# yuansliu/minicom

Measured on AMD Instinct MI355X. Metric: Mreads/s (sketch+index+overlap) on 150bp reads, 1/2/4/8 GPU; bit-exact decompress, higher is better.
Workload: dtype u64

## Files before the change

minicom_amd/csrc/api.hip:

```cpp
#include "mcom_dev.hpp"
#include "../../include/mcom_test.h"
#include <stdarg.h>
#include <stdlib.h>
#include <cxxabi.h>
#include <stdio.h>
#include <string.h>

int mcom_fail(mcom_ctx *ctx, int code, const char *fmt, ...)
{
	char buf[512];
	va_list ap;
	va_start(ap, fmt);
	vsnprintf(buf, sizeof buf, fmt, ap);
	va_end(ap);
	if (ctx) { ctx->err = buf; ctx->pin_wait.clear(); ctx->pin_off = 0; }
	return code;
}

#define MCOM_PIN_BYTES 4096
hipError_t mcom_d2h_async(mcom_ctx *ctx, void *dst, const void *src, size_t bytes)
{
	for (uint32_t q = 0; q < 8; ++q) {
		const mcom_ctx::ScanTotal &t = ctx->scan_last[(ctx->scan_last_at + 7u - q) % 8u];
		if (t.last && t.last == src && t.bytes == bytes && t.gen == ctx->launch_gen) { mcom_ctx::PinWait w{dst, 0, bytes}; w.from = ctx->scan_tot + t.slot; ctx->pin_wait.push_back(w); return hipSuccess; }
// ... 307 lines not shown
	if (!ctx) return MCOM_E_ARG;
	ctx->sketch_wave_only = wave_per_string == 1;
	ctx->sketch_ring64 = wave_per_string == 2;
	ctx->sketch_ring32_only = wave_per_string == 3;
	ctx->sketch_lane_always = wave_per_string >= 2;
	return MCOM_OK;
}
extern "C" int mcom_set_sketch_prefix_bits(mcom_ctx *ctx, int bits)
{
	if (!ctx || bits < 1 || bits > 30) return MCOM_E_ARG;
	ctx->sketch_prefix_bits = bits;
	return MCOM_OK;
}
extern "C" int mcom_set_claim_route(mcom_ctx *ctx, int route)
{
	if (!ctx || route < 0 || route > 3) return MCOM_E_ARG;
	ctx->claim_route = route;
	return MCOM_OK;
}
extern "C" int mcom_claim_fallbacks(const mcom_ctx *ctx) { return ctx ? (int)ctx->claim_fallbacks : 0; }
extern "C" int mcom_set_screen_route(mcom_ctx *ctx, int route)
{
	if (!ctx || route < 0 || route > 2) return MCOM_E_ARG;
	ctx->screen_route = route;
	return MCOM_OK;
}
extern "C" int mcom_screen_fallbacks(const mcom_ctx *ctx) { return ctx ? (int)ctx->screen_fallbacks : 0; }
extern "C" int mcom_set_lookup_route(mcom_ctx *ctx, int route)
{
	if (!ctx || route < 0 || route > 1) return MCOM_E_ARG;
	ctx->lookup_route = route;
	return MCOM_OK;
}
extern "C" int mcom_set_index_capacity(mcom_ctx *ctx, int entries)
{
	if (!ctx) return MCOM_E_ARG;
	ctx->cix_cap_set = entries >= 0; ctx->cix_cap = entries >= 0 ? (uint32_t)entries : 0u;
	return MCOM_OK;
}
```

minicom_amd/csrc/cindex.hip:

```cpp
#include "cindex.hpp"
#include <algorithm>

#define CX_THREADS 256
#define CX_ITEMS 24
#define CX_TILE (CX_THREADS * CX_ITEMS)

__global__ void k_cindex_blocks(int maxoff, const uint64_t *__restrict__ woff, uint32_t c0, uint32_t c1, uint64_t pos0, uint64_t n_blocks, uint32_t *__restrict__ first_contig)
{
	const uint32_t c = c0 + blockIdx.x * blockDim.x + threadIdx.x;
	if (c >= c1) return;
	const uint64_t a = woff[c] + (uint64_t)maxoff * c - pos0, b = woff[c + 1] + (uint64_t)maxoff * (c + 1) - pos0;
	for (uint64_t blk = (a + 255) >> 8; (blk << 8) < b && blk < n_blocks; ++blk) first_contig[blk] = c;
}

__device__ __forceinline__ uint32_t cx_tile(uint32_t b, uint32_t n_tiles) { const uint32_t per = (n_tiles + 7u) >> 3; return (b & 7u) * per + (b >> 3); }
static inline uint32_t cx_grid(uint32_t n_tiles) { return ((n_tiles + 7u) >> 3) << 3; }

struct CxSrc { const uint64_t *cbits, *coff, *woff; const uint32_t *first_contig; uint32_t c1; uint64_t pos0, n_pos; unsigned long long *head; };

struct CxWalk { uint32_t c; bool has; uint64_t p, np, lo, hi; };
__device__ __forceinline__ uint64_t cx_first(const CixGeom &g, const CxSrc &s, uint32_t c) { return s.woff[c] + (uint64_t)g.maxoff * c - s.pos0; }
__device__ __forceinline__ void cx_load(const CixGeom &g, const CxSrc &s, CxWalk &w)
{
	w.has = s.woff[w.c + 1] != s.woff[w.c];
	if (!w.has || w.p >= w.np) return;
	const uint64_t len = (s.woff[w.c + 1] - s.woff[w.c]) + (uint64_t)g.L - 1;
	const uint64_t q = (2 * len + 63) >> 6, i = (2 * w.p) >> 6;
	const uint64_t *src = s.cbits + s.coff[w.c] + i;
	const int sh = (int)((2 * w.p) & 63);
	const uint64_t w0 = src[0], w1 = src[1], w2 = i + 2 <= q ? src[2] : 0ull;
	w.lo = sh ? (w0 >> sh) | (w1 << (64 - sh)) : w0;
	w.hi = sh ? (w1 >> sh) | (w2 << (64 - sh)) : w1;
}
__device__ __forceinline__ void cx_seek(const CixGeom &g, const CxSrc &s, uint64_t gi, CxWalk &w)
{
	uint32_t c = s.first_contig[gi >> 8];
	while (c + 1 < s.c1 && cx_first(g, s, c + 1) <= gi) ++c;
	const uint64_t a = cx_first(g, s, c);
	w.c = c; w.p = gi - a; w.np = cx_first(g, s, c + 1) - a;
	cx_load(g, s, w);
}
__device__ __forceinline__ bool cx_step(const CixGeom &g, const CxSrc &s, CxWalk &w, uint32_t &key32, uint64_t &slot, uint32_t &digit)
{
	while (w.p >= w.np) {
		++w.c; w.p = 0; w.np = cx_first(g, s, w.c + 1) - cx_first(g, s, w.c);
		cx_load(g, s, w);
	}
	bool ok = w.has;
	if (ok && (w.p >> g.pbits)) { if (*(volatile unsigned long long*)(s.head + 1) == 0) s.head[1] = 1; ok = false; }
	if (ok) {
		const uint64_t key = w.lo & ((1ull << (2 * g.klen)) - 1);
		uint32_t own, part, h16;
		cix_hash(key, g.n_owners, g.n_parts, own, part, h16);
		key32 = (part << 16) | h16;
		digit = g.n_owners > 1 ? own : (part >> 8);
		slot = (cix_tag(key) << CIX_TAG_SHIFT) | ((uint64_t)w.c << g.pbits) | w.p;
	}
	w.lo = (w.lo >> 2) | (w.hi << 62); w.hi >>= 2; ++w.p;
	return ok;
}

__global__ __launch_bounds__(CX_THREADS) void k_cx_hist1(CixGeom g, CxSrc s, uint32_t *__restrict__ hist, uint32_t nblocks)
{
	__shared__ uint32_t h[256];
	const uint32_t tile = cx_tile(blockIdx.x, nblocks);
	if (tile >= nblocks) return;
	h[threadIdx.x] = 0;
	__syncthreads();
	uint64_t gi = (uint64_t)tile * CX_TILE + (uint64_t)threadIdx.x * CX_ITEMS;
	if (gi < s.n_pos) {
		CxWalk w; cx_seek(g, s, gi, w);
#pragma unroll 4
		for (int it = 0; it < CX_ITEMS && gi < s.n_pos; ++it, ++gi) {
			uint32_t k32, dg; uint64_t sl;
			if (cx_step(g, s, w, k32, sl, dg)) atomicAdd(&h[dg], 1u);
		}
	}
	__syncthreads();
	hist[(size_t)threadIdx.x * nblocks + tile] = h[threadIdx.x];
}

template <bool OWNERS>
__global__ __launch_bounds__(CX_THREADS) void k_cx_scatter1(CixGeom g, CxSrc s, const uint32_t *__restrict__ offs, uint32_t nblocks,
                                                            uint32_t *__restrict__ out_key, uint64_t *__restrict__ out_slot)
{
	__shared__ uint64_t st_slot[CX_TILE];
	__shared__ uint32_t st_key[CX_TILE];
	__shared__ uint8_t st_dig[OWNERS ? CX_TILE : 4];
	__shared__ uint32_t cnt[256], start[256], gofs[256], wsum[CX_THREADS / 64];
	const int tid = threadIdx.x, lane = tid & 63, wv = tid >> 6;
	const uint32_t tile = cx_tile(blockIdx.x, nblocks);
	if (tile >= nblocks) return;
	cnt[tid] = 0;
	__syncthreads();
	uint64_t gi = (uint64_t)tile * CX_TILE + (uint64_t)tid * CX_ITEMS;
	uint32_t k32[CX_ITEMS], rank[CX_ITEMS]; uint64_t sl[CX_ITEMS]; bool ok[CX_ITEMS]; uint8_t dg[CX_ITEMS];
	{
		CxWalk w; w.c = 0; w.has = false; w.p = w.np = w.lo = w.hi = 0;
		if (gi < s.n_pos) cx_seek(g, s, gi, w);
#pragma unroll
		for (int it = 0; it < CX_ITEMS; ++it, ++gi) {
			uint32_t d = 0;
			ok[it] = gi < s.n_pos && cx_step(g, s, w, k32[it], sl[it], d);
			dg[it] = (uint8_t)d;
			rank[it] = ok[it] ? atomicAdd(&cnt[d], 1u) : 0u;
		}
	}
	__syncthreads();
	{
		const uint32_t tot = cnt[tid];
		uint32_t v = tot;
#pragma unroll
		for (int d = 1; d < 64; d <<= 1) { const uint32_t t = __shfl_up(v, d, 64); if (lane >= d) v += t; }
		if (lane == 63) wsum[wv] = v;
		__syncthreads();
		uint32_t add = 0;
		for (int q = 0; q < wv; ++q) add += wsum[q];
		start[tid] = v + add - tot;
		gofs[tid] = offs[(size_t)tid * nblocks + tile];
	}
	__syncthreads();
#pragma unroll
	for (int it = 0; it < CX_ITEMS; ++it) if (ok[it]) {
		const uint32_t at = start[dg[it]] + rank[it];
		st_key[at] = k32[it]; st_slot[at] = sl[it];
		if (OWNERS) st_dig[at] = dg[it];
	}
	__syncthreads();
	const uint32_t total = start[255] + cnt[255];
	for (uint32_t q = tid; q < total; q += CX_THREADS) {
		const uint32_t d = OWNERS ? (uint32_t)st_dig[q] : st_key[q] >> 24;
		const size_t o = (size_t)gofs[d] + (q - start[d]);
		out_key[o] = st_key[q]; out_slot[o] = st_slot[q];
	}
}

struct CxTiles { uint32_t rs[257], tp[257]; };
__global__ void k_cx_regions(const uint32_t *__restrict__ key, uint32_t n, CxTiles *__restrict__ T)
{
	__shared__ uint32_t tl[257];
	const uint32_t v = threadIdx.x;
	uint32_t lo = 0, hi = n;
	if (v >= 256) lo = n;
	else while (lo < hi) { const uint32_t mid = lo + ((hi - lo) >> 1); if ((key[mid] >> 24) < v) lo = mid + 1; else hi = mid; }
	T->rs[v] = lo; tl[v] = lo;
	__syncthreads();
	if (v == 0) {
		uint32_t run = 0;
		for (int r = 0; r < 256; ++r) { T->tp[r] = run; run += (tl[r + 1] - tl[r] + CX_TILE - 1) / CX_TILE; }
		T->tp[256] = run;
	}
}
struct CxWhere { uint32_t r, t, nt, first, count; };
__device__ __forceinline__ bool cx_where(const CxTiles *__restrict__ T, uint32_t b, uint32_t *sh_tp, CxWhere &w)
{
	for (uint32_t q = threadIdx.x; q < 257; q += blockDim.x) sh_tp[q] = T->tp[q];
	__syncthreads();
	if (b >= sh_tp[256]) return false;
	uint32_t lo = 0, hi = 255;
	while (lo < hi) { const uint32_t mid = (lo + hi + 1) >> 1; if (sh_tp[mid] <= b) lo = mid; else hi = mid - 1; }
	w.r = lo; w.t = b - sh_tp[lo]; w.nt = sh_tp[lo + 1] - sh_tp[lo];
	const uint32_t a = T->rs[lo], e = T->rs[lo + 1];
	w.first = a + w.t * CX_TILE;
	w.count = e - w.first < (uint32_t)CX_TILE ? e - w.first : (uint32_t)CX_TILE;
	return true;
}
template <bool REGION>
__global__ __launch_bounds__(CX_THREADS) void k_cx_hist2(const uint32_t *__restrict__ key, uint32_t n, const CxTiles *__restrict__ T, uint32_t *__restrict__ hist, uint32_t nblocks)
{
	__shared__ uint32_t h[256], sh_tp[257];
	const uint32_t b = cx_tile(blockIdx.x, nblocks);
	if (b >= nblocks) return;
	h[threadIdx.x] = 0;
	uint32_t first, count; size_t at;
	if (REGION) {
		CxWhere w;
		if (!cx_where(T, b, sh_tp, w)) { hist[(size_t)256 * b + threadIdx.x] = 0; return; }
		first = w.first; count = w.count; at = (size_t)256 * sh_tp[w.r] + (size_t)threadIdx.x * w.nt + w.t;
	} else {
		__syncthreads();
		first = b * (uint32_t)CX_TILE; count = n - first < (uint32_t)CX_TILE ? n - first : (uint32_t)CX_TILE;
		at = (size_t)threadIdx.x * nblocks + b;
	}
#pragma unroll 4
	for (int it = 0; it < CX_ITEMS; ++it) {
		const uint32_t i = (uint32_t)it * CX_THREADS + threadIdx.x;
		if (i < count) atomicAdd(&h[(key[first + i] >> (REGION ? 16 : 24)) & 255u], 1u);
	}
	__syncthreads();
	hist[at] = h[threadIdx.x];
}
template <bool REGION>
__global__ __launch_bounds__(CX_THREADS) void k_cx_scatter2(const uint32_t *__restrict__ in_key, const uint64_t *__restrict__ in_slot, uint32_t n, const CxTiles *__restrict__ T,
                                                            const uint32_t *__restrict__ offs, uint32_t nblocks, uint32_t *__restrict__ out_key, uint64_t *__restrict__ out_slot)
{
	__shared__ uint64_t st_slot[CX_TILE];
	__shared__ uint32_t st_key[CX_TILE];
	__shared__ uint32_t cnt[256], start[256], gofs[256], wsum[CX_THREADS / 64], sh_tp[257];
	const int tid = threadIdx.x, lane = tid & 63, wv = tid >> 6;
	constexpr int SHIFT = REGION ? 16 : 24;
	const uint32_t b = cx_tile(blockIdx.x, nblocks);
	if (b >= nblocks) return;
	cnt[tid] = 0;
	uint32_t first, count; size_t at;
	if (REGION) {
		CxWhere w;
		if (!cx_where(T, b, sh_tp, w)) return;
		first = w.first; count = w.count; at = (size_t)256 * sh_tp[w.r] + (size_t)tid * w.nt + w.t;
	} else {
		__syncthreads();
		first = b * (uint32_t)CX_TILE; count = n - first < (uint32_t)CX_TILE ? n - first : (uint32_t)CX_TILE;
		at = (size_t)tid * nblocks + b;
	}
	uint32_t k32[CX_ITEMS], rank[CX_ITEMS]; uint64_t sl[CX_ITEMS];
#pragma unroll
	for (int it = 0; it < CX_ITEMS; ++it) {
		const uint32_t i = (uint32_t)it * CX_THREADS + tid;
		if (i < count) { k32[it] = in_key[first + i]; sl[it] = in_slot[first + i]; }
	}
#pragma unroll
	for (int it = 0; it < CX_ITEMS; ++it) {
		const uint32_t i = (uint32_t)it * CX_THREADS + tid;
		rank[it] = i < count ? atomicAdd(&cnt[(k32[it] >> SHIFT) & 255u], 1u) : 0u;
	}
	__syncthreads();
	{
		const uint32_t tot = cnt[tid];
		uint32_t v = tot;
#pragma unroll
		for (int d = 1; d < 64; d <<= 1) { const uint32_t t = __shfl_up(v, d, 64); if (lane >= d) v += t; }
		if (lane == 63) wsum[wv] = v;
		__syncthreads();
		uint32_t add = 0;
		for (int q = 0; q < wv; ++q) add += wsum[q];
		start[tid] = v + add - tot;
		gofs[tid] = offs[at];
	}
	__syncthreads();
#pragma unroll
	for (int it = 0; it < CX_ITEMS; ++it) {
		const uint32_t i = (uint32_t)it * CX_THREADS + tid;
		if (i < count) { const uint32_t p = start[(k32[it] >> SHIFT) & 255u] + rank[it]; st_key[p] = k32[it]; st_slot[p] = sl[it]; }
	}
	__syncthreads();
	for (uint32_t q = tid; q < count; q += CX_THREADS) {
		const uint32_t k = st_key[q], d = (k >> SHIFT) & 255u;
		const size_t o = (size_t)gofs[d] + (q - start[d]);
		out_key[o] = k; out_slot[o] = st_slot[q];
	}
}

__global__ void k_cx_pstart(const CxTiles *__restrict__ T, const uint32_t *__restrict__ offs, uint32_t n, uint32_t n_parts, uint32_t *__restrict__ pstart)
{
	const uint32_t v = blockIdx.x * blockDim.x + threadIdx.x;
	if (v > n_parts) return;
	const uint32_t r = v >> 8, d = v & 255u;
	uint32_t at = n;
	if (v < n_parts && r < 256) {
		const uint32_t nt = T->tp[r + 1] - T->tp[r];
		at = nt ? offs[(size_t)256 * T->tp[r] + (size_t)d * nt] : T->rs[r];
	}
	pstart[v] = at;
}
#define CA_THREADS 512
#define CA_BATCH 8
__global__ __launch_bounds__(CA_THREADS) void k_cx_assemble(const uint32_t *__restrict__ key, const uint64_t *__restrict__ slot, const uint32_t *__restrict__ pstart,
                                                            uint32_t n_parts, uint32_t NL, unsigned long long *__restrict__ head, uint64_t ext_cap,
                                                            const uint8_t *__restrict__ redo)
{
	extern __shared__ uint32_t sm[];
	if (!redo[blockIdx.x]) return;
	uint32_t *cnt = sm;
	int32_t *carry = (int32_t*)(sm + NL);
	uint32_t *runb = sm + 2 * (size_t)NL;
	__shared__ int32_t agg_sum[CA_THREADS / 64], agg_min[CA_THREADS / 64];
	__shared__ uint32_t red[CA_THREADS / 64];
	__shared__ int32_t s_c0;
	const uint32_t part = blockIdx.x;
// ... 266 lines not shown
static inline size_t cx_al(size_t b) { return (b + 255) & ~(size_t)255; }

extern "C" int mcom_cindex_entries(mcom_ctx *ctx, const uint64_t *d_cbits, const uint64_t *d_coff, const uint64_t *d_woff, uint32_t n_contigs,
                                   uint32_t c0, uint32_t c1, int L, int ininumdict, uint64_t geom, uint32_t *d_key, uint64_t *d_slot, uint64_t cap,
                                   uint64_t *h_counts)
{
	if (!ctx || !h_counts) return MCOM_E_ARG;
	CixGeom g;
	if (L < 1 || L > 256 || cix_geom(L, ininumdict, g)) return mcom_fail(ctx, MCOM_E_ARG, "bad dictionary layout");
	cix_unpack(geom, g);
	for (uint32_t q = 0; q < g.n_owners; ++q) h_counts[q] = 0;
	if (g.n_parts < 1 || g.n_lines < 1) return mcom_fail(ctx, MCOM_E_ARG, "bad contig index geometry");
	if (c0 > c1 || c1 > n_contigs) return mcom_fail(ctx, MCOM_E_ARG, "bad contig range");
	g.pbits = cix_pbits(n_contigs);
	if (c0 == c1) return MCOM_OK;
	if (!d_cbits || !d_coff || !d_woff || !d_key || !d_slot) return mcom_fail(ctx, MCOM_E_ARG, "null device pointer");
	McomProfScope ps_(ctx, PROF_CINDEX_BUILD);
	uint64_t w01[2] = {0, 0};
	MCOM_HIP(ctx, mcom_d2h_async(ctx, &w01[0], d_woff + c0, 8));
	MCOM_HIP(ctx, mcom_d2h_async(ctx, &w01[1], d_woff + c1, 8));
	MCOM_HIP(ctx, mcom_stream_sync(ctx));
	const uint64_t n_pos = (w01[1] - w01[0]) ? (w01[1] - w01[0]) + (uint64_t)(c1 - c0) * (uint64_t)g.maxoff : 0;
	if (n_pos >= (1ull << 32)) return mcom_fail(ctx, MCOM_E_ARG, "too many contig positions");
	if (n_pos > cap) return mcom_fail(ctx, MCOM_E_OVERFLOW, "contig index entries: room for %llu, %llu positions", (unsigned long long)cap, (unsigned long long)n_pos);
	if (!n_pos) return MCOM_OK;
	const uint32_t nblocks = (uint32_t)((n_pos + CX_TILE - 1) / CX_TILE);
	const uint64_t blocks256 = (n_pos + 255) / 256;
	const size_t hist_b = cx_al((size_t)256 * nblocks * 4 + 64), scr_b = cx_al(mcom_scan_scratch_elems((size_t)256 * nblocks + 2) * 4 + 1024), map_b = cx_al((size_t)blocks256 * 4 + 4);
	char *tmp = nullptr;
	if (mcom_dmalloc(&tmp, hist_b + scr_b + map_b + 2 * 256) != hipSuccess) return mcom_fail(ctx, MCOM_E_NOMEM, "contig index: scratch");
	struct Guard { mcom_ctx *c; char *p; ~Guard() { (void)hipStreamSynchronize(c->stream); mcom_dfree(p); } } guard{ctx, tmp};
	uint32_t *hist = (uint32_t*)tmp, *scr = (uint32_t*)(tmp + hist_b), *first_contig = (uint32_t*)(tmp + hist_b + scr_b);
	unsigned long long *head = (unsigned long long*)(tmp + hist_b + scr_b + map_b);
	MCOM_HIP(ctx, hipMemsetAsync(head, 0, 16, ctx->stream));
	const uint64_t pos0 = w01[0] + (uint64_t)g.maxoff * c0;
	MCOM_LAUNCH(k_cindex_blocks, dim3((c1 - c0 + 255) / 256), dim3(256), 0, ctx->stream, g.maxoff, d_woff, c0, c1, pos0, blocks256, first_contig);
	MCOM_LAUNCH_CHECK(ctx);
	const CxSrc src{d_cbits, d_coff, d_woff, first_contig, c1, pos0, n_pos, head};
	MCOM_LAUNCH(k_cx_hist1, dim3(cx_grid(nblocks)), dim3(CX_THREADS), 0, ctx->stream, g, src, hist, nblocks);
	MCOM_LAUNCH_CHECK(ctx);
	MCOM_HIP(ctx, hipMemsetAsync(hist + (size_t)256 * nblocks, 0, 4, ctx->stream));
	int rc;
	if ((rc = mcom_scan_u32(ctx, hist, hist, (size_t)256 * nblocks + 1, scr))) return rc;
	if (g.n_owners > 1) MCOM_LAUNCH(k_cx_scatter1<true>, dim3(cx_grid(nblocks)), dim3(CX_THREADS), 0, ctx->stream, g, src, hist, nblocks, d_key, d_slot);
	else MCOM_LAUNCH(k_cx_scatter1<false>, dim3(cx_grid(nblocks)), dim3(CX_THREADS), 0, ctx->stream, g, src, hist, nblocks, d_key, d_slot);
	MCOM_LAUNCH_CHECK(ctx);
	std::vector<uint32_t> st(g.n_owners + 1, 0);
	if (g.n_owners > 1) { for (uint32_t q = 1; q < g.n_owners; ++q) MCOM_HIP(ctx, hipMemcpyAsync(&st[q], hist + (size_t)q * nblocks, 4, hipMemcpyDeviceToHost, ctx->stream)); }
	MCOM_HIP(ctx, hipMemcpyAsync(&st[g.n_owners], hist + (size_t)256 * nblocks, 4, hipMemcpyDeviceToHost, ctx->stream));
	uint64_t hd[2] = {0, 0};
	MCOM_HIP(ctx, hipMemcpyAsync(hd, head, 16, hipMemcpyDeviceToHost, ctx->stream));
	MCOM_HIP(ctx, mcom_stream_sync(ctx));
	if (hd[1]) return mcom_fail(ctx, MCOM_E_ARG, "contig index: a contig of this set of %u contigs is longer than 2^%d bases", n_contigs, g.pbits);
	for (uint32_t q = 0; q < g.n_owners; ++q) h_counts[q] = (uint64_t)st[q + 1] - st[q];
	return MCOM_OK;
}

extern "C" int mcom_cindex_partition(mcom_ctx *ctx, uint32_t *d_key, uint64_t *d_slot, uint64_t n_ent64, int grouped, uint32_t *d_key_tmp, uint64_t *d_slot_tmp,
                                     int L, int ininumdict, uint64_t geom, uint32_t *d_pstart, const uint32_t **d_key_sorted, const uint64_t **d_slot_sorted)
{
	if (!ctx || !d_key_sorted || !d_slot_sorted) return MCOM_E_ARG;
	CixGeom g;
	if (L < 1 || L > 256 || cix_geom(L, ininumdict, g)) return mcom_fail(ctx, MCOM_E_ARG, "bad dictionary layout");
	cix_unpack(geom, g);
	if (!d_pstart || g.n_parts < 1 || g.n_lines < 1) return mcom_fail(ctx, MCOM_E_ARG, "bad contig index buffers");
	if (n_ent64 >= (1ull << 32)) return mcom_fail(ctx, MCOM_E_ARG, "too many contig index entries for one share");
	if (n_ent64 && (!d_key || !d_slot || !d_key_tmp || !d_slot_tmp)) return mcom_fail(ctx, MCOM_E_ARG, "null device pointer");
	const uint32_t n_ent = (uint32_t)n_ent64;
	McomProfScope ps_(ctx, PROF_CINDEX_BUILD);
	const uint32_t nbA = std::max<uint32_t>(1, (uint32_t)(((size_t)n_ent + CX_TILE - 1) / CX_TILE));
	const uint32_t nbR = nbA + 256;
	const size_t hist_b = cx_al((size_t)256 * nbR * 4 + 64), scr_b = cx_al(mcom_scan_scratch_elems((size_t)256 * nbR + 2) * 4 + 1024);
	char *tmp = nullptr;
	if (mcom_dmalloc(&tmp, hist_b + scr_b + cx_al(sizeof(CxTiles)) + 256) != hipSuccess) return mcom_fail(ctx, MCOM_E_NOMEM, "contig index: scratch");
	struct Guard { mcom_ctx *c; char *p; ~Guard() { (void)hipStreamSynchronize(c->stream); mcom_dfree(p); } } guard{ctx, tmp};
	uint32_t *hist = (uint32_t*)tmp, *scr = (uint32_t*)(tmp + hist_b);
	CxTiles *tiles = (CxTiles*)(tmp + hist_b + scr_b);
	const uint32_t *skey = d_key; const uint64_t *sslot = d_slot;
	int rc;
	uint32_t *ik = d_key, *ok = d_key_tmp; uint64_t *is = d_slot, *os = d_slot_tmp;
	if (n_ent && !grouped) {
		MCOM_LAUNCH(k_cx_hist2<false>, dim3(cx_grid(nbA)), dim3(CX_THREADS), 0, ctx->stream, ik, n_ent, (const CxTiles*)nullptr, hist, nbA);
		MCOM_LAUNCH_CHECK(ctx);
		if ((rc = mcom_scan_u32(ctx, hist, hist, (size_t)256 * nbA, scr))) return rc;
		MCOM_LAUNCH(k_cx_scatter2<false>, dim3(cx_grid(nbA)), dim3(CX_THREADS), 0, ctx->stream, ik, is, n_ent, (const CxTiles*)nullptr, hist, nbA, ok, os);
		MCOM_LAUNCH_CHECK(ctx);
		std::swap(ik, ok); std::swap(is, os);
	}
	MCOM_LAUNCH(k_cx_regions, dim3(1), dim3(257), 0, ctx->stream, ik, n_ent, tiles);
	MCOM_LAUNCH_CHECK(ctx);
	if (n_ent) {
		MCOM_LAUNCH(k_cx_hist2<true>, dim3(cx_grid(nbR)), dim3(CX_THREADS), 0, ctx->stream, ik, n_ent, (const CxTiles*)tiles, hist, nbR);
		MCOM_LAUNCH_CHECK(ctx);
		if ((rc = mcom_scan_u32(ctx, hist, hist, (size_t)256 * nbR, scr))) return rc;
		MCOM_LAUNCH(k_cx_scatter2<true>, dim3(cx_grid(nbR)), dim3(CX_THREADS), 0, ctx->stream, ik, is, n_ent, (const CxTiles*)tiles, hist, nbR, ok, os);
		MCOM_LAUNCH_CHECK(ctx);
		std::swap(ik, ok); std::swap(is, os);
		skey = ik; sslot = is;
	}
	MCOM_LAUNCH(k_cx_pstart, dim3((g.n_parts + 1 + 255) / 256), dim3(256), 0, ctx->stream, (const CxTiles*)tiles, hist, n_ent, g.n_parts, d_pstart);
	MCOM_LAUNCH_CHECK(ctx);
	*d_key_sorted = skey; *d_slot_sorted = sslot;
	return MCOM_OK;
}

extern "C" int mcom_cindex_assemble(mcom_ctx *ctx, const uint32_t *d_key_sorted, const uint64_t *d_slot_sorted, const uint32_t *d_pstart, int L, int ininumdict,
                                    uint64_t geom, uint64_t *d_keys, uint64_t n_words)
{
	if (!ctx) return MCOM_E_ARG;
	CixGeom g;
	if (L < 1 || L > 256 || cix_geom(L, ininumdict, g)) return mcom_fail(ctx, MCOM_E_ARG, "bad dictionary layout");
	cix_unpack(geom, g);
	const uint64_t main_lines = (uint64_t)g.n_parts * g.n_lines;
	if (!d_keys || !d_pstart || g.n_parts < 1 || g.n_lines < 1 || n_words < CIX_HEAD_WORDS + 8 * (main_lines + 1)) return mcom_fail(ctx, MCOM_E_ARG, "bad contig index buffers");
	const uint64_t ext_cap = (n_words - CIX_HEAD_WORDS) / 8 - main_lines;
	McomProfScope ps_(ctx, PROF_CINDEX_BUILD);
	MCOM_HIP(ctx, hipMemsetAsync(d_keys, 0, CIX_HEAD_WORDS * 8, ctx->stream));
	uint8_t *redo = nullptr;
	if (mcom_dmalloc(&redo, (size_t)g.n_parts + 256) != hipSuccess) return mcom_fail(ctx, MCOM_E_NOMEM, "contig index: scratch");
	struct Guard { mcom_ctx *c; uint8_t *p; ~Guard() { (void)hipStreamSynchronize(c->stream); mcom_dfree(p); } } guard{ctx, redo};
	const size_t lds = (size_t)3 * g.n_lines * 4;
	if (lds > 150 * 1024) return mcom_fail(ctx, MCOM_E_ARG, "contig index: partitions of %u lines", g.n_lines);
	MCOM_HIP(ctx, hipMemsetAsync(redo, 0, g.n_parts, ctx->stream));
	MCOM_LAUNCH(k_cx_assemble_sorted, dim3(g.n_parts), dim3(CS_THREADS), 0, ctx->stream, d_key_sorted, d_slot_sorted, d_pstart, g.n_parts, g.n_lines, (unsigned long long*)d_keys, ext_cap, redo,
	                   ctx->cix_cap_set ? std::min<uint32_t>(ctx->cix_cap, CS_CAP) : (uint32_t)CS_CAP);
	MCOM_LAUNCH_CHECK(ctx);
	MCOM_HIP(ctx, hipFuncSetAttribute((const void*)k_cx_assemble, hipFuncAttributeMaxDynamicSharedMemorySize, (int)lds));
	MCOM_LAUNCH(k_cx_assemble, dim3(g.n_parts), dim3(CA_THREADS), lds, ctx->stream, d_key_sorted, d_slot_sorted, d_pstart, g.n_parts, g.n_lines, (unsigned long long*)d_keys, ext_cap, redo);
// ... 48 lines not shown
```

minicom_amd/csrc/mcom_dev.hpp:

```cpp
#pragma once
#include <hip/hip_runtime.h>
#include <stdint.h>
#include <stddef.h>
#include <map>
#include <string>
#include <vector>
#include "../../include/mcom.h"

enum McomProfId { PROF_CLASSIFY_PACK = 0, PROF_SKETCH_READS, PROF_RADIX_PASS, PROF_SKETCH_CONTIGS, PROF_FIND_NEXT,
                  PROF_DICT_BUILD, PROF_REALIGN_WINDOWS, PROF_CONSENSUS, PROF_CINDEX_BUILD, PROF_REALIGN_READS, PROF_COUNT };
struct McomProfSpan { int id; hipEvent_t a, b; };

struct mcom_ctx {
	int device;
	hipStream_t stream;
	std::string err;
	void *ws; size_t ws_bytes;
	int n_cu;
	bool prof_on = false;
	std::vector<McomProfSpan> prof_open;
	double prof_ms[PROF_COUNT] = {0};
	uint64_t prof_calls[PROF_COUNT] = {0};
	int prof_cur = PROF_COUNT;
	std::map<std::pair<int, const void *>, uint64_t> prof_kernels;
	uint32_t seg_cap = 0; uint64_t sort_overflow_segments = 0;
	uint64_t sketch_strings = 0;
	bool cix_cap_set = false; uint32_t cix_cap = 0;
	uint32_t bs_cap = 0;
	bool sketch_wave_only = false;
	bool sketch_lane_always = false;
	bool sketch_ring64 = false, sketch_ring32_only = false; int sketch_prefix_bits = 14;
	unsigned long long *scan_parts = nullptr; uint32_t scan_epoch = 0; volatile unsigned int *poison = nullptr; unsigned int *d_poison = nullptr;
	enum { SCAN_TOTALS = 64 };
	unsigned long long *scan_tot = nullptr, *d_scan_tot = nullptr;
	struct ScanTotal { const void *last; uint32_t bytes, slot, gen; } scan_last[8] = {}; uint32_t scan_last_at = 0, launch_gen = 1;
	int claim_route = 0; uint64_t claim_fallbacks = 0;
	unsigned int *screen_flag = nullptr;
	std::vector<void*> free_later;
	int screen_route = 0; uint64_t screen_fallbacks = 0;
	int lookup_route = 0;
	int verify_hash_bits = 64;
	struct ScreenArgs { const uint64_t *sgbits; size_t n_sg; int L, ininumdict, maxsearch, n_shares, share; } screen_args = {};
	enum { ZPOOL_BYTES = 64 * 1024 };
	unsigned char *zpool = nullptr; size_t zpool_used = 0; int zpool_half = 0;
	struct PinWait { void *dst; size_t off, bytes; const void *from = nullptr; };
	unsigned char *pin = nullptr; size_t pin_off = 0;
	std::vector<PinWait> pin_wait;
};

hipEvent_t mcom_prof_event_get();
void mcom_prof_event_put(hipEvent_t e);
struct McomProfScope {
	mcom_ctx *ctx; int idx;
	McomProfScope(mcom_ctx *c, int id) : ctx(c), idx(-1) {
		if (!c->prof_on) return;
		McomProfSpan s; s.id = id;
		if (!(s.a = mcom_prof_event_get())) return;
		if (!(s.b = mcom_prof_event_get())) { mcom_prof_event_put(s.a); return; }
		(void)hipEventRecord(s.a, c->stream);
		c->prof_open.push_back(s); idx = (int)c->prof_open.size() - 1;
// ... 166 lines not shown
```

minicom_amd/hip.py:

```python
from __future__ import annotations

import ctypes as C
import os
import re

import numpy as np

HERE = os.path.dirname(os.path.abspath(__file__))
MM_DTYPE = np.dtype([("x", "<u8"), ("y", "<u8")])


class McomError(RuntimeError):
    pass


class DecodeSrc(C.Structure):
    _fields_ = [("d_text", C.c_void_p), ("text_bytes", C.c_uint64), ("d_line_start", C.c_void_p), ("verbatim", C.c_int),
                ("d_ref", C.c_void_p), ("ref_bytes", C.c_uint64), ("ref_const", C.c_int),
                ("d_cid", C.c_void_p), ("d_pos", C.c_void_p), ("d_coff", C.c_void_p), ("n_contigs", C.c_uint64),
                ("d_dir", C.c_void_p), ("dir_bytes", C.c_uint64)]


DECODE_F_BOUNDS, DECODE_F_LINE, DECODE_F_DUP, DECODE_F_DEST = 1, 2, 4, 8

# ... 486 lines not shown
        self.lib.mcom_cindex_entries.restype = C.c_int
        self.lib.mcom_cindex_entries.argtypes = [C.c_void_p] * 4 + [C.c_uint32] * 3 + [C.c_int, C.c_int, u64, C.c_void_p, C.c_void_p, u64, C.POINTER(u64)]
        self.lib.mcom_cindex_place.restype = C.c_int
        self.lib.mcom_cindex_place.argtypes = [C.c_void_p, C.c_void_p, C.c_void_p, u64, C.c_int, C.c_void_p, C.c_void_p, C.c_int, C.c_int, u64, C.c_void_p, u64]
        n_contigs = int(coff.shape[0])
        ne, share, geom0, nw = u64(), u64(), u64(), u64()
        self._check(self.lib.mcom_cindex_plan_shared(int(n_windows), n_contigs, L, ininumdict, ranks, 0, C.byref(ne), C.byref(share), C.byref(geom0), C.byref(nw)))
        cap = int(ne.value) + 1
        key = torch.empty(cap, dtype=torch.int32, device=self.device)
        slot = torch.empty(cap, dtype=torch.int64, device=self.device)
        counts = (u64 * ranks)()
        self._check(self.lib.mcom_cindex_entries(self._h, self._p(cbits, torch.int64), self._p(coff, torch.int64), self._p(woff, torch.int64), n_contigs, 0, n_contigs,
                                                 L, ininumdict, geom0.value, self._p(key), self._p(slot), cap, counts))
        out, at = [], 0
        for q in range(ranks):
            g, nwq = u64(), u64()
            self._check(self.lib.mcom_cindex_plan_shared(int(n_windows), n_contigs, L, ininumdict, ranks, q, C.byref(ne), C.byref(share), C.byref(g), C.byref(nwq)))
            n = int(counts[q])
            words = int(nwq.value)
            for attempt in range(5):
                k, sl = key[at:at + n].clone(), slot[at:at + n].clone()
                kt, st = torch.empty(n + 1, dtype=torch.int32, device=self.device), torch.empty(n + 1, dtype=torch.int64, device=self.device)
                keys = torch.empty(words, dtype=torch.int64, device=self.device)
                rc = self.lib.mcom_cindex_place(self._h, self._p(k), self._p(sl), n, 0, self._p(kt), self._p(st), L, ininumdict, g.value, self._p(keys), words)
                if rc != -4:
                    break
                words += max(words, 8 * (int(ne.value) // 7 + 1024))
            self._check(rc)
            self.sync()
            out.append((keys, g.value))
            at += n
        return out

    def set_lookup_route(self, route: int):
        self.lib.mcom_set_lookup_route.restype = C.c_int; self.lib.mcom_set_lookup_route.argtypes = [C.c_void_p, C.c_int]
        self._check(self.lib.mcom_set_lookup_route(self._h, route))

    def dicts_eligible(self, dicts, sgbits, maxsearch: int):
        torch = _torch()
        el = torch.zeros(max(int(sgbits.shape[0]), 1), dtype=torch.int32, device=self.device)
        self._check(self.lib.mcom_dicts_eligible(self._h, dicts._h, self._p(sgbits, torch.int64), maxsearch, self._p(el)))
        return el

    def dicts_screen(self, sgbits, L: int, maxsearch: int, ininumdict: int = 0) -> bool:
        torch = _torch()
        out = C.c_int(0)
        self._check(self.lib.mcom_dicts_screen(self._h, self._p(sgbits, torch.int64), int(sgbits.shape[0]), L, ininumdict, maxsearch, C.byref(out)))
        return bool(out.value)

    def realign_pass_reads(self, cindex, sgbits, sgflag, cbits, coff, woff, L: int, thr: int, ininumdict: int = 0, elig=None,
                           stats: bool = False):
        torch = _torch()
        keys, lg = cindex
        n_sg = int(sgbits.shape[0])
        claim = torch.empty(max(n_sg, 1), dtype=torch.int64, device=self.device)
        st = torch.zeros(3, dtype=torch.int64, device=self.device) if stats else None
        self._check(self.lib.mcom_realign_pass_reads(self._h, self._p(keys), lg, self._p(sgbits, torch.int64),
                                                     self._p(sgflag, torch.uint8), self._p(elig), n_sg, self._p(cbits, torch.int64),
                                                     self._p(coff, torch.int64), self._p(woff, torch.int64), int(coff.shape[0]), L,
                                                     ininumdict, thr, self._p(claim), self._p(st)))
        return claim[:n_sg], st

    def scan_u64(self, x):
        torch = _torch()
        out = torch.empty_like(x)
        self._check(self.lib.mcom_scan_u64(self._h, self._p(x, torch.int64), self._p(out), int(x.shape[0])))
# ... 737 lines not shown
```

Before: 554.0.

## Stage contig bits into LDS for cindex scatter and widen scatter blocks

The scatter pass of the contig index now first stages each tile's contig start offsets and the packed 2-bit words it needs into shared memory, reusing the pass's own staging arrays. It then walks k-mers from LDS, falling back to the global-memory walk when a tile spans too many contigs or words. Both scatter kernels move from 256 to 512 threads per block with fewer items per thread, and counters and route knobs are added for testing. The aim is to cut repeated scattered global loads of woff, coff and cbits during the walk. The cost is an extra staging phase with barriers and atomics, plus possibly lower occupancy at 512 threads with the same LDS footprint.

```diff
diff --git a/minicom_amd/csrc/api.hip b/minicom_amd/csrc/api.hip
--- a/minicom_amd/csrc/api.hip
+++ b/minicom_amd/csrc/api.hip
@@ -363,6 +363,18 @@
 	ctx->lookup_route = route;
 	return MCOM_OK;
 }
+extern "C" int mcom_set_cindex_route(mcom_ctx *ctx, int route)
+{
+	if (!ctx || route < 0 || route > 2) return MCOM_E_ARG;
+	ctx->cx_route = route;
+	return MCOM_OK;
+}
+extern "C" int mcom_cindex_tiles(const mcom_ctx *ctx, uint64_t *tiles, uint64_t *from_global)
+{
+	if (!ctx || !tiles || !from_global) return MCOM_E_ARG;
+	*tiles = ctx->cx_tiles; *from_global = ctx->cx_tiles_global;
+	return MCOM_OK;
+}
 extern "C" int mcom_set_index_capacity(mcom_ctx *ctx, int entries)
 {
 	if (!ctx) return MCOM_E_ARG;
diff --git a/minicom_amd/csrc/cindex.hip b/minicom_amd/csrc/cindex.hip
--- a/minicom_amd/csrc/cindex.hip
+++ b/minicom_amd/csrc/cindex.hip
@@ -4,6 +4,8 @@
 #define CX_THREADS 256
 #define CX_ITEMS 24
 #define CX_TILE (CX_THREADS * CX_ITEMS)
+#define CX_STHREADS 512
+#define CX_SITEMS (CX_TILE / CX_STHREADS)
 
 __global__ void k_cindex_blocks(int maxoff, const uint64_t *__restrict__ woff, uint32_t c0, uint32_t c1, uint64_t pos0, uint64_t n_blocks, uint32_t *__restrict__ first_contig)
 {
@@ -19,35 +21,66 @@
 struct CxSrc { const uint64_t *cbits, *coff, *woff; const uint32_t *first_contig; uint32_t c1; uint64_t pos0, n_pos; unsigned long long *head; };
 
 struct CxWalk { uint32_t c; bool has; uint64_t p, np, lo, hi; };
-__device__ __forceinline__ uint64_t cx_first(const CixGeom &g, const CxSrc &s, uint32_t c) { return s.woff[c] + (uint64_t)g.maxoff * c - s.pos0; }
-__device__ __forceinline__ void cx_load(const CixGeom &g, const CxSrc &s, CxWalk &w)
-{
-	w.has = s.woff[w.c + 1] != s.woff[w.c];
+struct CxGlobal {
+	const CixGeom &g; const CxSrc &s;
+	__device__ __forceinline__ uint64_t first(uint32_t c) const { return s.woff[c] + (uint64_t)g.maxoff * c - s.pos0; }
+	__device__ __forceinline__ uint64_t nwin(uint32_t c) const { return s.woff[c + 1] - s.woff[c]; }
+	__device__ __forceinline__ uint32_t seek(uint64_t gi) const
+	{
+		uint32_t c = s.first_contig[gi >> 8];
+		while (c + 1 < s.c1 && first(c + 1) <= gi) ++c;
+		return c;
+	}
+	__device__ __forceinline__ void words(uint32_t c, uint64_t i, bool third, uint64_t &w0, uint64_t &w1, uint64_t &w2) const
+	{
+		const uint64_t *src = s.cbits + s.coff[c] + i;
+		w0 = src[0]; w1 = src[1]; w2 = third ? src[2] : 0ull;
+	}
+};
+struct CxStaged {
+	const uint32_t *first_, *rel; const uint64_t *wd; uint32_t cA, nc, maxoff;
+	__device__ __forceinline__ uint64_t first(uint32_t c) const { return first_[c - cA]; }
+	__device__ __forceinline__ uint64_t nwin(uint32_t c) const { return (uint64_t)(first_[c + 1 - cA] - first_[c - cA]) - maxoff; }
+	__device__ __forceinline__ uint32_t seek(uint64_t gi) const
+	{
+		uint32_t lo = 0, hi = nc - 1;
+		while (lo < hi) { const uint32_t mid = (lo + hi + 1) >> 1; if (first_[mid] <= gi) lo = mid; else hi = mid - 1; }
+		return cA + lo;
+	}
+	__device__ __forceinline__ void words(uint32_t c, uint64_t i, bool third, uint64_t &w0, uint64_t &w1, uint64_t &w2) const
+	{
+		const uint32_t j = rel[c - cA] + (uint32_t)i;
+		w0 = wd[j]; w1 = wd[j + 1]; w2 = third ? wd[j + 2] : 0ull;
+	}
+};
+template <class S> __device__ __forceinline__ void cx_load(const CixGeom &g, const S &s, CxWalk &w)
+{
+	const uint64_t nw = s.nwin(w.c);
+	w.has = nw != 0;
 	if (!w.has || w.p >= w.np) return;
-	const uint64_t len = (s.woff[w.c + 1] - s.woff[w.c]) + (uint64_t)g.L - 1;
+	const uint64_t len = nw + (uint64_t)g.L - 1;
 	const uint64_t q = (2 * len + 63) >> 6, i = (2 * w.p) >> 6;
-	const uint64_t *src = s.cbits + s.coff[w.c] + i;
 	const int sh = (int)((2 * w.p) & 63);
-	const uint64_t w0 = src[0], w1 = src[1], w2 = i + 2 <= q ? src[2] : 0ull;
+	uint64_t w0, w1, w2;
+	s.words(w.c, i, i + 2 <= q, w0, w1, w2);
 	w.lo = sh ? (w0 >> sh) | (w1 << (64 - sh)) : w0;
 	w.hi = sh ? (w1 >> sh) | (w2 << (64 - sh)) : w1;
 }
-__device__ __forceinline__ void cx_seek(const CixGeom &g, const CxSrc &s, uint64_t gi, CxWalk &w)
-{
-	uint32_t c = s.first_contig[gi >> 8];
-	while (c + 1 < s.c1 && cx_first(g, s, c + 1) <= gi) ++c;
-	const uint64_t a = cx_first(g, s, c);
-	w.c = c; w.p = gi - a; w.np = cx_first(g, s, c + 1) - a;
+template <class S> __device__ __forceinline__ void cx_seek(const CixGeom &g, const S &s, uint64_t gi, CxWalk &w)
+{
+	const uint32_t c = s.seek(gi);
+	const uint64_t a = s.first(c);
+	w.c = c; w.p = gi - a; w.np = s.first(c + 1) - a;
 	cx_load(g, s, w);
 }
-__device__ __forceinline__ bool cx_step(const CixGeom &g, const CxSrc &s, CxWalk &w, uint32_t &key32, uint64_t &slot, uint32_t &digit)
+template <class S> __device__ __forceinline__ bool cx_step(const CixGeom &g, const S &s, unsigned long long *head, CxWalk &w, uint32_t &key32, uint64_t &slot, uint32_t &digit)
 {
 	while (w.p >= w.np) {
-		++w.c; w.p = 0; w.np = cx_first(g, s, w.c + 1) - cx_first(g, s, w.c);
+		++w.c; w.p = 0; w.np = s.first(w.c + 1) - s.first(w.c);
 		cx_load(g, s, w);
 	}
 	bool ok = w.has;
-	if (ok && (w.p >> g.pbits)) { if (*(volatile unsigned long long*)(s.head + 1) == 0) s.head[1] = 1; ok = false; }
+	if (ok && (w.p >> g.pbits)) { if (*(volatile unsigned long long*)(head + 1) == 0) head[1] = 1; ok = false; }
 	if (ok) {
 		const uint64_t key = w.lo & ((1ull << (2 * g.klen)) - 1);
 		uint32_t own, part, h16;
@@ -60,6 +93,65 @@
 	return ok;
 }
 
+#define CX_SC 512
+#define CX_SW 1536
+static_assert(CX_SC % CX_STHREADS == 0 && 2 * CX_SC + 1 <= CX_TILE && CX_SW + 3 <= CX_TILE, "the staged source lies inside pass 1's staging arrays");
+struct CxStageMeta { unsigned long long wlo, whi; uint32_t nc; };
+template <int T> __device__ __forceinline__ bool cx_stage(const CixGeom &g, const CxSrc &s, uint64_t t0, uint32_t cap_c, uint32_t cap_w,
+                                         uint32_t *sfirst, uint32_t *srel, uint64_t *swd, CxStageMeta *m, CxStaged &st)
+{
+	if (cap_c == 0) return false;
+	const uint32_t tid = threadIdx.x;
+	const uint64_t t1 = t0 + CX_TILE < s.n_pos ? t0 + CX_TILE : s.n_pos;
+	const uint32_t cA = s.first_contig[t0 >> 8];
+	const uint32_t nav = s.c1 - cA < cap_c ? s.c1 - cA : cap_c;
+	if (tid == 0) { m->nc = 0; m->wlo = ~0ull; m->whi = 0; }
+	for (uint32_t j = tid; j <= nav; j += T) sfirst[j] = (uint32_t)(s.woff[cA + j] + (uint64_t)g.maxoff * (cA + j) - s.pos0);
+	__syncthreads();
+	for (uint32_t j = tid + 1; j <= nav; j += T) if (sfirst[j] >= t1 && sfirst[j - 1] < t1) m->nc = j;
+	__syncthreads();
+	const uint32_t nc = m->nc;
+	if (nc == 0 || sfirst[0] > t0) return false;
+	uint64_t co[CX_SC / T];
+#pragma unroll
+	for (int k = 0; k < CX_SC / T; ++k) {
+		const uint32_t j = tid + k * T;
+		co[k] = 0;
+		if (j < nc) {
+			co[k] = s.coff[cA + j];
+			const uint64_t f = sfirst[j], np = sfirst[j + 1] - sfirst[j];
+			const uint64_t plo = f < t0 ? t0 - f : 0;
+			if (np > (uint64_t)g.maxoff && plo < np) {
+				const uint64_t phi = (np < t1 - f ? np : t1 - f) - 1;
+				const uint64_t len = np - g.maxoff + (uint64_t)g.L - 1, q = (2 * len + 63) >> 6;
+				const uint64_t lo = (2 * plo) >> 6, hi = ((2 * phi) >> 6) + 2 <= q ? ((2 * phi) >> 6) + 2 : q;
+				atomicMin(&m->wlo, (unsigned long long)(co[k] + lo));
+				atomicMax(&m->whi, (unsigned long long)(co[k] + hi));
+			}
+		}
+	}
+	__syncthreads();
+	const uint64_t wlo = m->wlo, whi = m->whi;
+	const uint64_t nwd = whi >= wlo ? whi - wlo + 1 : 0;
+	if (nwd > cap_w) return false;
+#pragma unroll
+	for (int k = 0; k < CX_SC / T; ++k) { const uint32_t j = tid + k * T; if (j < nc) srel[j] = (uint32_t)(co[k] - wlo); }
+	for (uint32_t j = tid; j < (uint32_t)nwd; j += T) swd[j] = s.cbits[wlo + j];
+	__syncthreads();
+	st.first_ = sfirst; st.rel = srel; st.wd = swd; st.cA = cA; st.nc = nc; st.maxoff = (uint32_t)g.maxoff;
+	return true;
+}
+
+template <class S> __device__ __forceinline__ void cx_hist_walk(const CixGeom &g, const S &src, unsigned long long *head, uint64_t gi, uint64_t n_pos, uint32_t *h)
+{
+	if (gi >= n_pos) return;
+	CxWalk w; cx_seek(g, src, gi, w);
+#pragma unroll 4
+	for (int it = 0; it < CX_ITEMS && gi < n_pos; ++it, ++gi) {
+		uint32_t k32, dg; uint64_t sl;
+		if (cx_step(g, src, head, w, k32, sl, dg)) atomicAdd(&h[dg], 1u);
+	}
+}
 __global__ __launch_bounds__(CX_THREADS) void k_cx_hist1(CixGeom g, CxSrc s, uint32_t *__restrict__ hist, uint32_t nblocks)
 {
 	__shared__ uint32_t h[256];
@@ -67,68 +159,75 @@
 	if (tile >= nblocks) return;
 	h[threadIdx.x] = 0;
 	__syncthreads();
-	uint64_t gi = (uint64_t)tile * CX_TILE + (uint64_t)threadIdx.x * CX_ITEMS;
-	if (gi < s.n_pos) {
-		CxWalk w; cx_seek(g, s, gi, w);
-#pragma unroll 4
-		for (int it = 0; it < CX_ITEMS && gi < s.n_pos; ++it, ++gi) {
-			uint32_t k32, dg; uint64_t sl;
-			if (cx_step(g, s, w, k32, sl, dg)) atomicAdd(&h[dg], 1u);
-		}
-	}
+	const uint64_t t0 = (uint64_t)tile * CX_TILE, gi = t0 + (uint64_t)threadIdx.x * CX_ITEMS;
+	cx_hist_walk(g, CxGlobal{g, s}, s.head, gi, s.n_pos, h);
 	__syncthreads();
 	hist[(size_t)threadIdx.x * nblocks + tile] = h[threadIdx.x];
 }
 
+template <class S, int N> __device__ __forceinline__ void cx_scatter_walk(const CixGeom &g, const S &src, unsigned long long *head, uint64_t gi, uint64_t n_pos, uint32_t *cnt,
+                                                                          uint32_t (&k32)[N], uint64_t (&sl)[N], uint32_t (&rank)[N], bool (&ok)[N], uint8_t (&dg)[N])
+{
+	CxWalk w; w.c = 0; w.has = false; w.p = w.np = w.lo = w.hi = 0;
+	if (gi < n_pos) cx_seek(g, src, gi, w);
+#pragma unroll
+	for (int it = 0; it < N; ++it, ++gi) {
+		uint32_t d = 0;
+		ok[it] = gi < n_pos && cx_step(g, src, head, w, k32[it], sl[it], d);
+		dg[it] = (uint8_t)d;
+		rank[it] = ok[it] ? atomicAdd(&cnt[d], 1u) : 0u;
+	}
+}
 template <bool OWNERS>
-__global__ __launch_bounds__(CX_THREADS) void k_cx_scatter1(CixGeom g, CxSrc s, const uint32_t *__restrict__ offs, uint32_t nblocks,
-                                                            uint32_t *__restrict__ out_key, uint64_t *__restrict__ out_slot)
+__global__ __launch_bounds__(CX_STHREADS) void k_cx_scatter1(CixGeom g, CxSrc s, const uint32_t *__restrict__ offs, uint32_t nblocks,
+                                                            uint32_t *__restrict__ out_key, uint64_t *__restrict__ out_slot, uint32_t cap_c, uint32_t cap_w)
 {
 	__shared__ uint64_t st_slot[CX_TILE];
 	__shared__ uint32_t st_key[CX_TILE];
 	__shared__ uint8_t st_dig[OWNERS ? CX_TILE : 4];
-	__shared__ uint32_t cnt[256], start[256], gofs[256], wsum[CX_THREADS / 64];
+	__shared__ uint32_t cnt[256], start[256], gofs[256], wsum[4];
 	const int tid = threadIdx.x, lane = tid & 63, wv = tid >> 6;
 	const uint32_t tile = cx_tile(blockIdx.x, nblocks);
 	if (tile >= nblocks) return;
-	cnt[tid] = 0;
-	__syncthreads();
-	uint64_t gi = (uint64_t)tile * CX_TILE + (uint64_t)tid * CX_ITEMS;
-	uint32_t k32[CX_ITEMS], rank[CX_ITEMS]; uint64_t sl[CX_ITEMS]; bool ok[CX_ITEMS]; uint8_t dg[CX_ITEMS];
-	{
-		CxWalk w; w.c = 0; w.has = false; w.p = w.np = w.lo = w.hi = 0;
-		if (gi < s.n_pos) cx_seek(g, s, gi, w);
-#pragma unroll
-		for (int it = 0; it < CX_ITEMS; ++it, ++gi) {
-			uint32_t d = 0;
-			ok[it] = gi < s.n_pos && cx_step(g, s, w, k32[it], sl[it], d);
-			dg[it] = (uint8_t)d;
-			rank[it] = ok[it] ? atomicAdd(&cnt[d], 1u) : 0u;
-		}
-	}
-	__syncthreads();
-	{
-		const uint32_t tot = cnt[tid];
-		uint32_t v = tot;
-#pragma unroll
-		for (int d = 1; d < 64; d <<= 1) { const uint32_t t = __shfl_up(v, d, 64); if (lane >= d) v += t; }
-		if (lane == 63) wsum[wv] = v;
-		__syncthreads();
-		uint32_t add = 0;
-		for (int q = 0; q < wv; ++q) add += wsum[q];
-		start[tid] = v + add - tot;
-		gofs[tid] = offs[(size_t)tid * nblocks + tile];
-	}
-	__syncthreads();
-#pragma unroll
-	for (int it = 0; it < CX_ITEMS; ++it) if (ok[it]) {
+	if (tid < 256) cnt[tid] = 0;
+	__syncthreads();
+	const uint64_t t0 = (uint64_t)tile * CX_TILE, gi = t0 + (uint64_t)tid * CX_SITEMS;
+	uint32_t k32[CX_SITEMS], rank[CX_SITEMS]; uint64_t sl[CX_SITEMS]; bool ok[CX_SITEMS]; uint8_t dg[CX_SITEMS];
+	{
+		CxStaged st;
+		if (cx_stage<CX_STHREADS>(g, s, t0, cap_c, cap_w, st_key, st_key + CX_SC + 1, st_slot, (CxStageMeta*)(st_slot + CX_SW), st)) cx_scatter_walk(g, st, s.head, gi, s.n_pos, cnt, k32, sl, rank, ok, dg);
+		else {
+			if (tid == 0) atomicAdd(s.head + 2, 1ull);
+			cx_scatter_walk(g, CxGlobal{g, s}, s.head, gi, s.n_pos, cnt, k32, sl, rank, ok, dg);
+		}
+	}
+	__syncthreads();
+	{
+		uint32_t tot = 0, v = 0;
+		if (tid < 256) {
+			tot = v = cnt[tid];
+#pragma unroll
+			for (int d = 1; d < 64; d <<= 1) { const uint32_t t = __shfl_up(v, d, 64); if (lane >= d) v += t; }
+			if (lane == 63) wsum[wv] = v;
+		}
+		__syncthreads();
+		if (tid < 256) {
+			uint32_t add = 0;
+			for (int q = 0; q < wv; ++q) add += wsum[q];
+			start[tid] = v + add - tot;
+			gofs[tid] = offs[(size_t)tid * nblocks + tile];
+		}
+	}
+	__syncthreads();
+#pragma unroll
+	for (int it = 0; it < CX_SITEMS; ++it) if (ok[it]) {
 		const uint32_t at = start[dg[it]] + rank[it];
 		st_key[at] = k32[it]; st_slot[at] = sl[it];
 		if (OWNERS) st_dig[at] = dg[it];
 	}
 	__syncthreads();
 	const uint32_t total = start[255] + cnt[255];
-	for (uint32_t q = tid; q < total; q += CX_THREADS) {
+	for (uint32_t q = tid; q < total; q += CX_STHREADS) {
 		const uint32_t d = OWNERS ? (uint32_t)st_dig[q] : st_key[q] >> 24;
 		const size_t o = (size_t)gofs[d] + (q - start[d]);
 		out_key[o] = st_key[q]; out_slot[o] = st_slot[q];
@@ -191,17 +290,17 @@
 	hist[at] = h[threadIdx.x];
 }
 template <bool REGION>
-__global__ __launch_bounds__(CX_THREADS) void k_cx_scatter2(const uint32_t *__restrict__ in_key, const uint64_t *__restrict__ in_slot, uint32_t n, const CxTiles *__restrict__ T,
+__global__ __launch_bounds__(CX_STHREADS) void k_cx_scatter2(const uint32_t *__restrict__ in_key, const uint64_t *__restrict__ in_slot, uint32_t n, const CxTiles *__restrict__ T,
                                                             const uint32_t *__restrict__ offs, uint32_t nblocks, uint32_t *__restrict__ out_key, uint64_t *__restrict__ out_slot)
 {
 	__shared__ uint64_t st_slot[CX_TILE];
 	__shared__ uint32_t st_key[CX_TILE];
-	__shared__ uint32_t cnt[256], start[256], gofs[256], wsum[CX_THREADS / 64], sh_tp[257];
+	__shared__ uint32_t cnt[256], start[256], gofs[256], wsum[4], sh_tp[257];
 	const int tid = threadIdx.x, lane = tid & 63, wv = tid >> 6;
 	constexpr int SHIFT = REGION ? 16 : 24;
 	const uint32_t b = cx_tile(blockIdx.x, nblocks);
 	if (b >= nblocks) return;
-	cnt[tid] = 0;
+	if (tid < 256) cnt[tid] = 0;
 	uint32_t first, count; size_t at;
 	if (REGION) {
 		CxWhere w;
@@ -212,38 +311,42 @@
 		first = b * (uint32_t)CX_TILE; count = n - first < (uint32_t)CX_TILE ? n - first : (uint32_t)CX_TILE;
 		at = (size_t)tid * nblocks + b;
 	}
-	uint32_t k32[CX_ITEMS], rank[CX_ITEMS]; uint64_t sl[CX_ITEMS];
-#pragma unroll
-	for (int it = 0; it < CX_ITEMS; ++it) {
-		const uint32_t i = (uint32_t)it * CX_THREADS + tid;
+	uint32_t k32[CX_SITEMS], rank[CX_SITEMS]; uint64_t sl[CX_SITEMS];
+#pragma unroll
+	for (int it = 0; it < CX_SITEMS; ++it) {
+		const uint32_t i = (uint32_t)it * CX_STHREADS + tid;
 		if (i < count) { k32[it] = in_key[first + i]; sl[it] = in_slot[first + i]; }
 	}
 #pragma unroll
-	for (int it = 0; it < CX_ITEMS; ++it) {
-		const uint32_t i = (uint32_t)it * CX_THREADS + tid;
+	for (int it = 0; it < CX_SITEMS; ++it) {
+		const uint32_t i = (uint32_t)it * CX_STHREADS + tid;
 		rank[it] = i < count ? atomicAdd(&cnt[(k32[it] >> SHIFT) & 255u], 1u) : 0u;
 	}
 	__syncthreads();
 	{
-		const uint32_t tot = cnt[tid];
-		uint32_t v = tot;
-#pragma unroll
-		for (int d = 1; d < 64; d <<= 1) { const uint32_t t = __shfl_up(v, d, 64); if (lane >= d) v += t; }
-		if (lane == 63) wsum[wv] = v;
-		__syncthreads();
-		uint32_t add = 0;
-		for (int q = 0; q < wv; ++q) add += wsum[q];
-		start[tid] = v + add - tot;
-		gofs[tid] = offs[at];
-	}
-	__syncthreads();
-#pragma unroll
-	for (int it = 0; it < CX_ITEMS; ++it) {
-		const uint32_t i = (uint32_t)it * CX_THREADS + tid;
+		uint32_t tot = 0, v = 0;
+		if (tid < 256) {
+			tot = v = cnt[tid];
+#pragma unroll
+			for (int d = 1; d < 64; d <<= 1) { const uint32_t t = __shfl_up(v, d, 64); if (lane >= d) v += t; }
+			if (lane == 63) wsum[wv] = v;
+		}
+		__syncthreads();
+		if (tid < 256) {
+			uint32_t add = 0;
+			for (int q = 0; q < wv; ++q) add += wsum[q];
+			start[tid] = v + add - tot;
+			gofs[tid] = offs[at];
+		}
+	}
+	__syncthreads();
+#pragma unroll
+	for (int it = 0; it < CX_SITEMS; ++it) {
+		const uint32_t i = (uint32_t)it * CX_STHREADS + tid;
 		if (i < count) { const uint32_t p = start[(k32[it] >> SHIFT) & 255u] + rank[it]; st_key[p] = k32[it]; st_slot[p] = sl[it]; }
 	}
 	__syncthreads();
-	for (uint32_t q = tid; q < count; q += CX_THREADS) {
+	for (uint32_t q = tid; q < count; q += CX_STHREADS) {
 		const uint32_t k = st_key[q], d = (k >> SHIFT) & 255u;
 		const size_t o = (size_t)gofs[d] + (q - start[d]);
 		out_key[o] = k; out_slot[o] = st_slot[q];
@@ -576,7 +679,8 @@
 	struct Guard { mcom_ctx *c; char *p; ~Guard() { (void)hipStreamSynchronize(c->stream); mcom_dfree(p); } } guard{ctx, tmp};
 	uint32_t *hist = (uint32_t*)tmp, *scr = (uint32_t*)(tmp + hist_b), *first_contig = (uint32_t*)(tmp + hist_b + scr_b);
 	unsigned long long *head = (unsigned long long*)(tmp + hist_b + scr_b + map_b);
-	MCOM_HIP(ctx, hipMemsetAsync(head, 0, 16, ctx->stream));
+	MCOM_HIP(ctx, hipMemsetAsync(head, 0, 32, ctx->stream));
+	const uint32_t cap_c = ctx->cx_route == 1 ? 0u : ctx->cx_route == 2 ? 4u : (uint32_t)CX_SC, cap_w = ctx->cx_route == 2 ? 200u : (uint32_t)CX_SW;
 	const uint64_t pos0 = w01[0] + (uint64_t)g.maxoff * c0;
 	MCOM_LAUNCH(k_cindex_blocks, dim3((c1 - c0 + 255) / 256), dim3(256), 0, ctx->stream, g.maxoff, d_woff, c0, c1, pos0, blocks256, first_contig);
 	MCOM_LAUNCH_CHECK(ctx);
@@ -586,15 +690,16 @@
 	MCOM_HIP(ctx, hipMemsetAsync(hist + (size_t)256 * nblocks, 0, 4, ctx->stream));
 	int rc;
 	if ((rc = mcom_scan_u32(ctx, hist, hist, (size_t)256 * nblocks + 1, scr))) return rc;
-	if (g.n_owners > 1) MCOM_LAUNCH(k_cx_scatter1<true>, dim3(cx_grid(nblocks)), dim3(CX_THREADS), 0, ctx->stream, g, src, hist, nblocks, d_key, d_slot);
-	else MCOM_LAUNCH(k_cx_scatter1<false>, dim3(cx_grid(nblocks)), dim3(CX_THREADS), 0, ctx->stream, g, src, hist, nblocks, d_key, d_slot);
+	if (g.n_owners > 1) MCOM_LAUNCH(k_cx_scatter1<true>, dim3(cx_grid(nblocks)), dim3(CX_STHREADS), 0, ctx->stream, g, src, hist, nblocks, d_key, d_slot, cap_c, cap_w);
+	else MCOM_LAUNCH(k_cx_scatter1<false>, dim3(cx_grid(nblocks)), dim3(CX_STHREADS), 0, ctx->stream, g, src, hist, nblocks, d_key, d_slot, cap_c, cap_w);
 	MCOM_LAUNCH_CHECK(ctx);
 	std::vector<uint32_t> st(g.n_owners + 1, 0);
 	if (g.n_owners > 1) { for (uint32_t q = 1; q < g.n_owners; ++q) MCOM_HIP(ctx, hipMemcpyAsync(&st[q], hist + (size_t)q * nblocks, 4, hipMemcpyDeviceToHost, ctx->stream)); }
 	MCOM_HIP(ctx, hipMemcpyAsync(&st[g.n_owners], hist + (size_t)256 * nblocks, 4, hipMemcpyDeviceToHost, ctx->stream));
-	uint64_t hd[2] = {0, 0};
-	MCOM_HIP(ctx, hipMemcpyAsync(hd, head, 16, hipMemcpyDeviceToHost, ctx->stream));
+	uint64_t hd[4] = {0, 0, 0, 0};
+	MCOM_HIP(ctx, hipMemcpyAsync(hd, head, 32, hipMemcpyDeviceToHost, ctx->stream));
 	MCOM_HIP(ctx, mcom_stream_sync(ctx));
+	ctx->cx_tiles += nblocks; ctx->cx_tiles_global += hd[2];
 	if (hd[1]) return mcom_fail(ctx, MCOM_E_ARG, "contig index: a contig of this set of %u contigs is longer than 2^%d bases", n_contigs, g.pbits);
 	for (uint32_t q = 0; q < g.n_owners; ++q) h_counts[q] = (uint64_t)st[q + 1] - st[q];
 	return MCOM_OK;
@@ -627,7 +732,7 @@
 		MCOM_LAUNCH(k_cx_hist2<false>, dim3(cx_grid(nbA)), dim3(CX_THREADS), 0, ctx->stream, ik, n_ent, (const CxTiles*)nullptr, hist, nbA);
 		MCOM_LAUNCH_CHECK(ctx);
 		if ((rc = mcom_scan_u32(ctx, hist, hist, (size_t)256 * nbA, scr))) return rc;
-		MCOM_LAUNCH(k_cx_scatter2<false>, dim3(cx_grid(nbA)), dim3(CX_THREADS), 0, ctx->stream, ik, is, n_ent, (const CxTiles*)nullptr, hist, nbA, ok, os);
+		MCOM_LAUNCH(k_cx_scatter2<false>, dim3(cx_grid(nbA)), dim3(CX_STHREADS), 0, ctx->stream, ik, is, n_ent, (const CxTiles*)nullptr, hist, nbA, ok, os);
 		MCOM_LAUNCH_CHECK(ctx);
 		std::swap(ik, ok); std::swap(is, os);
 	}
@@ -637,7 +742,7 @@
 		MCOM_LAUNCH(k_cx_hist2<true>, dim3(cx_grid(nbR)), dim3(CX_THREADS), 0, ctx->stream, ik, n_ent, (const CxTiles*)tiles, hist, nbR);
 		MCOM_LAUNCH_CHECK(ctx);
 		if ((rc = mcom_scan_u32(ctx, hist, hist, (size_t)256 * nbR, scr))) return rc;
-		MCOM_LAUNCH(k_cx_scatter2<true>, dim3(cx_grid(nbR)), dim3(CX_THREADS), 0, ctx->stream, ik, is, n_ent, (const CxTiles*)tiles, hist, nbR, ok, os);
+		MCOM_LAUNCH(k_cx_scatter2<true>, dim3(cx_grid(nbR)), dim3(CX_STHREADS), 0, ctx->stream, ik, is, n_ent, (const CxTiles*)tiles, hist, nbR, ok, os);
 		MCOM_LAUNCH_CHECK(ctx);
 		std::swap(ik, ok); std::swap(is, os);
 		skey = ik; sslot = is;
diff --git a/minicom_amd/csrc/mcom_dev.hpp b/minicom_amd/csrc/mcom_dev.hpp
--- a/minicom_amd/csrc/mcom_dev.hpp
+++ b/minicom_amd/csrc/mcom_dev.hpp
@@ -26,6 +26,7 @@
 	uint32_t seg_cap = 0; uint64_t sort_overflow_segments = 0;
 	uint64_t sketch_strings = 0;
 	bool cix_cap_set = false; uint32_t cix_cap = 0;
+	int cx_route = 0; uint64_t cx_tiles = 0, cx_tiles_global = 0;
 	uint32_t bs_cap = 0;
 	bool sketch_wave_only = false;
 	bool sketch_lane_always = false;
diff --git a/minicom_amd/hip.py b/minicom_amd/hip.py
--- a/minicom_amd/hip.py
+++ b/minicom_amd/hip.py
@@ -542,6 +542,36 @@
             at += n
         return out
 
+    def cindex_entries(self, cbits, coff, woff, n_windows: int, L: int, c0: int = 0, c1=None, ranks: int = 1, ininumdict: int = 0):
+        torch = _torch()
+        u64 = C.c_uint64
+        self.lib.mcom_cindex_plan_shared.restype = C.c_int
+        self.lib.mcom_cindex_plan_shared.argtypes = [u64, C.c_uint32, C.c_int, C.c_int, C.c_int, C.c_int] + [C.POINTER(u64)] * 4
+        self.lib.mcom_cindex_entries.restype = C.c_int
+        self.lib.mcom_cindex_entries.argtypes = [C.c_void_p] * 4 + [C.c_uint32] * 3 + [C.c_int, C.c_int, u64, C.c_void_p, C.c_void_p, u64, C.POINTER(u64)]
+        n_contigs = int(coff.shape[0])
+        c1 = n_contigs if c1 is None else c1
+        ne, share, geom0, nw = u64(), u64(), u64(), u64()
+        self._check(self.lib.mcom_cindex_plan_shared(int(n_windows), n_contigs, L, ininumdict, ranks, 0, C.byref(ne), C.byref(share), C.byref(geom0), C.byref(nw)))
+        cap = int(ne.value) + 1
+        key = torch.empty(cap, dtype=torch.int32, device=self.device)
+        slot = torch.empty(cap, dtype=torch.int64, device=self.device)
+        counts = (u64 * ranks)()
+        self._check(self.lib.mcom_cindex_entries(self._h, self._p(cbits, torch.int64), self._p(coff, torch.int64), self._p(woff, torch.int64), n_contigs, c0, c1,
+                                                 L, ininumdict, geom0.value, self._p(key), self._p(slot), cap, counts))
+        counts = [int(v) for v in counts]
+        return key[:sum(counts)], slot[:sum(counts)], counts, int(geom0.value)
+
+    def set_cindex_route(self, route: int):
+        self.lib.mcom_set_cindex_route.restype = C.c_int; self.lib.mcom_set_cindex_route.argtypes = [C.c_void_p, C.c_int]
+        self._check(self.lib.mcom_set_cindex_route(self._h, route))
+
+    def cindex_tiles(self):
+        t, f = C.c_uint64(), C.c_uint64()
+        self.lib.mcom_cindex_tiles.restype = C.c_int; self.lib.mcom_cindex_tiles.argtypes = [C.c_void_p, C.POINTER(C.c_uint64), C.POINTER(C.c_uint64)]
+        self._check(self.lib.mcom_cindex_tiles(self._h, C.byref(t), C.byref(f)))
+        return int(t.value), int(f.value)
+
     def set_lookup_route(self, route: int):
         self.lib.mcom_set_lookup_route.restype = C.c_int; self.lib.mcom_set_lookup_route.argtypes = [C.c_void_p, C.c_int]
         self._check(self.lib.mcom_set_lookup_route(self._h, route))
```

After: 551.5. Within noise of the previous version (-0.5%).
